# m13ammed/6D-Pose-Estimation-for-Unseen-Categories

Hardware: AMD Instinct MI355X
Metric: RGB-D crops/sec (fwd+bwd), 1024 pts, at 1/2/4/8 MI355X; pose err vs ref (higher is better)
Workload: dtype fp32; 1 GPU; configs[1] shape: B=32 synthetic 640x480 RGB-D crops, 1024 pts, training step fwd+bwd on 1 GPU (global batch 32); execution=hip-graph, crop formation overlapped, global_batch=32, points_per_crop=1024, cad_points=1024, precision=model fp32 (f32 MFMA); crop geometry / C_gt normal equations fp64, parallelism=dp1

## Files before the change

### 6d-pose-estimation-for-unseen-categories_amd/csrc/spectral.hip

```cpp
#include "common.hpp"
#include "mfma_tile.hpp"

namespace {

constexpr int kRows = 64;
constexpr int kKC = 64;

using pk::f32x4;

__device__ __forceinline__ f32x4 mfma4(float a, float b, f32x4 c) {
  return __builtin_amdgcn_mfma_f32_16x16x4f32(a, b, c, 0, 0, 0);
}

constexpr int kCPB = 4;
__global__ __launch_bounds__(256) void spec_reduce_mfma_kernel(const float* __restrict__ x, int ldx,
                                                               const float* __restrict__ mass,
                                                               const float* __restrict__ evecs, int N, int S,
                                                               float* __restrict__ part) {
  __shared__ float4 red[4][kKC * kKC / 4];
  const int s = blockIdx.x, b = blockIdx.y, tid = threadIdx.x;
  const int w = tid >> 6, l = tid & 63, u = l & 15, g = l >> 4;
  const float* __restrict__ phi = evecs + (int64_t)b * N * kKC;
  const float* __restrict__ xb = x + (int64_t)b * N * ldx;
  const float* __restrict__ mb = mass ? mass + (int64_t)b * N : nullptr;
  const int r0 = s * kCPB * kRows;
  const int nch = min(kCPB, (N - r0 + kRows - 1) / kRows);
  float4 pv[4], xv[4];
  float wv[4];
  auto load = [&](int ch) {
    const int rw = r0 + ch * kRows + 16 * w;
#pragma unroll
    for (int q = 0; q < 4; ++q) {
      const int r = rw + 4 * q + g;
      const int rc = r < N ? r : N - 1;
      pv[q] = reinterpret_cast<const float4*>(phi + (int64_t)rc * kKC)[u];
      xv[q] = reinterpret_cast<const float4*>(xb + (int64_t)rc * ldx)[u];
      wv[q] = mb ? mb[rc] : 1.f;
    }
  };
  f32x4 acc[4][4];
#pragma unroll
  for (int kt = 0; kt < 4; ++kt)
#pragma unroll
    for (int ct = 0; ct < 4; ++ct) acc[kt][ct] = f32x4{0.f, 0.f, 0.f, 0.f};
  load(0);
  for (int ch = 0; ch < nch; ++ch) {
    const int rw = r0 + ch * kRows + 16 * w;
    float a[4][4], xs[4][4];
#pragma unroll
    for (int q = 0; q < 4; ++q) {
      const bool ok = rw + 4 * q + g < N;
      const float wr = ok ? wv[q] : 0.f;
      a[q][0] = pv[q].x, a[q][1] = pv[q].y, a[q][2] = pv[q].z, a[q][3] = pv[q].w;
      xs[q][0] = mb ? xv[q].x * wr : (ok ? xv[q].x : 0.f);
      xs[q][1] = mb ? xv[q].y * wr : (ok ? xv[q].y : 0.f);
      xs[q][2] = mb ? xv[q].z * wr : (ok ? xv[q].z : 0.f);
      xs[q][3] = mb ? xv[q].w * wr : (ok ? xv[q].w : 0.f);
    }
    if (ch + 1 < nch) load(ch + 1);
#pragma unroll
    for (int q = 0; q < 4; ++q)
#pragma unroll
      for (int kt = 0; kt < 4; ++kt)
#pragma unroll
        for (int ct = 0; ct < 4; ++ct) acc[kt][ct] = mfma4(a[q][kt], xs[q][ct], acc[kt][ct]);
  }
#pragma unroll
  for (int kt = 0; kt < 4; ++kt)
#pragma unroll
    for (int rr = 0; rr < 4; ++rr)
      red[w][(4 * (4 * g + rr) + kt) * (kKC / 4) + u] =
          make_float4(acc[kt][0][rr], acc[kt][1][rr], acc[kt][2][rr], acc[kt][3][rr]);
  __syncthreads();
  float4* __restrict__ o = reinterpret_cast<float4*>(part + ((int64_t)b * S + s) * kKC * kKC);
#pragma unroll
  for (int j = 0; j < kKC * kKC / 4 / 256; ++j) {
    const int e = tid + 256 * j;
    const float4 v0 = red[0][e], v1 = red[1][e], v2 = red[2][e], v3 = red[3][e];
    o[e] = make_float4(((v0.x + v1.x) + v2.x) + v3.x, ((v0.y + v1.y) + v2.y) + v3.y, ((v0.z + v1.z) + v2.z) + v3.z,
                       ((v0.w + v1.w) + v2.w) + v3.w);
  }
}

__global__ __launch_bounds__(1024) void spec_combine4_kernel(float* __restrict__ part, int S,
                                                             const float* __restrict__ evals,
                                                             float* __restrict__ t, int clamp_t, int write_t,
                                                             float* __restrict__ raw, float* __restrict__ scaled,
                                                             const float* __restrict__ saved, int want_gt) {
  __shared__ double gsum[16][kKC];
  const int b = blockIdx.x, y = blockIdx.y, tid = threadIdx.x;
  const int c = tid & 63, k = 16 * y + (tid >> 6);
  const float* pb = part + (int64_t)b * S * kKC * kKC + k * kKC + c;
  const float tc = clamp_t ? fmaxf(t[c], 1e-8f) : t[c];
  double v = 0.0;
  int s = 0;
  for (; s + 8 <= S; s += 8) {
    float ld[8];
#pragma unroll
    for (int q = 0; q < 8; ++q) ld[q] = pb[(int64_t)(s + q) * kKC * kKC];
#pragma unroll
    for (int q = 0; q < 8; ++q) v += (double)ld[q];
  }
  for (; s < S; ++s) v += (double)pb[(int64_t)s * kKC * kKC];
  const float lam = evals[b * kKC + k];
  const float E = expf(-lam * tc);
  const int64_t o = (int64_t)b * kKC * kKC + k * kKC + c;
  const float vf = (float)v;
  if (raw) raw[o] = vf;
  scaled[o] = E * vf;
  if (write_t && b == 0 && y == 0 && tid < kKC) t[c] = tc;
  if (want_gt) {
    gsum[tid >> 6][c] = -(double)lam * (double)E * ((double)saved[o] * v);
    __syncthreads();
    if (tid < kKC) {
      double a = 0.0;
#pragma unroll
      for (int q = 0; q < 16; ++q) a += gsum[q][c];
      part[(int64_t)b * S * kKC * kKC + (16 * y) * kKC + c] = (float)a;
    }
  }
}

struct SpecFuse {
  const float* part;
  int S, clamp_t, write_t, pad;
  const float* evals;
  float* t;
  float* raw;
};

template <bool FUSED>
__global__ __launch_bounds__(256) void spec_expand_mfma_kernel(const float* __restrict__ evecs,
                                                               const float* __restrict__ coef,
                                                               const float* __restrict__ mass, int N,
                                                               float* __restrict__ y, int ldy, int accumulate,
                                                               const float* __restrict__ gtb, int64_t gt_stride,
                                                               float* __restrict__ gt, SpecFuse fz) {
  __shared__ float4 scoef[kKC * kKC / 4];
  const int3 lb = pk::xcd_block3();
  const int tile = lb.x, b = lb.y, tid = threadIdx.x;
  const int w = tid >> 6, l = tid & 63, u = l & 15, g = l >> 4;
  if constexpr (FUSED) {
    constexpr int PER = kKC * kKC / 4 / 256;
    const float* pb = fz.part + (int64_t)b * fz.S * kKC * kKC;
    double v[PER][4];
#pragma unroll
    for (int j = 0; j < PER; ++j)
#pragma unroll
      for (int q = 0; q < 4; ++q) v[j][q] = 0.0;
    for (int s0 = 0; s0 < fz.S; ++s0) {
      float4 ld[PER];
#pragma unroll
      for (int j = 0; j < PER; ++j) ld[j] = reinterpret_cast<const float4*>(pb + (int64_t)s0 * kKC * kKC)[tid + 256 * j];
#pragma unroll
      for (int j = 0; j < PER; ++j) {
        v[j][0] += (double)ld[j].x;
        v[j][1] += (double)ld[j].y;
        v[j][2] += (double)ld[j].z;
        v[j][3] += (double)ld[j].w;
      }
    }
#pragma unroll
    for (int j = 0; j < PER; ++j) {
      const int e = tid + 256 * j, k = e >> 4, c4 = e & 15;
      const float lam = fz.evals[b * kKC + k];
      float o[4], r[4];
#pragma unroll
      for (int q = 0; q < 4; ++q) {
        const int c = 4 * c4 + q;
        const float tc = fz.clamp_t ? fmaxf(fz.t[c], 1e-8f) : fz.t[c];
        const float E = expf(-lam * tc);
        r[q] = (float)v[j][q];
        o[q] = E * r[q];
      }
      scoef[e] = make_float4(o[0], o[1], o[2], o[3]);
      if (tile == 0 && fz.raw != nullptr)
        reinterpret_cast<float4*>(fz.raw + (int64_t)b * kKC * kKC)[e] = make_float4(r[0], r[1], r[2], r[3]);
    }
    if (fz.write_t && tile == 0 && b == 0 && tid < kKC) fz.t[tid] = fmaxf(fz.t[tid], 1e-8f);
  } else {
    const float* __restrict__ cb = coef + (int64_t)b * kKC * kKC;
    float4 cv[kKC * kKC / 4 / 256];
#pragma unroll
    for (int j = 0; j < kKC * kKC / 4 / 256; ++j) cv[j] = reinterpret_cast<const float4*>(cb)[tid + 256 * j];
#pragma unroll
    for (int j = 0; j < kKC * kKC / 4 / 256; ++j) scoef[tid + 256 * j] = cv[j];
  }
  const int rw = tile * 64 + 16 * w;
  const float* __restrict__ phi = evecs + (int64_t)b * N * kKC;
  float4 pv[4];
  {
    const int r = rw + u < N ? rw + u : N - 1;
#pragma unroll
    for (int t = 0; t < 4; ++t) pv[t] = reinterpret_cast<const float4*>(phi + (int64_t)r * kKC)[4 * t + g];
  }
  float wr[4];
  float4 old[4];
#pragma unroll
  for (int rr = 0; rr < 4; ++rr) {
    const int r = rw + 4 * g + rr < N ? rw + 4 * g + rr : N - 1;
    wr[rr] = mass ? mass[(int64_t)b * N + r] : 1.f;
    old[rr] = accumulate ? reinterpret_cast<const float4*>(y + ((int64_t)b * N + r) * ldy)[u]
                         : make_float4(0.f, 0.f, 0.f, 0.f);
  }
  __syncthreads();
  f32x4 acc[4];
#pragma unroll
  for (int ct = 0; ct < 4; ++ct) acc[ct] = f32x4{0.f, 0.f, 0.f, 0.f};
#pragma unroll
  for (int t = 0; t < 4; ++t) {
    const float pa[4] = {pv[t].x, pv[t].y, pv[t].z, pv[t].w};
#pragma unroll
    for (int e = 0; e < 4; ++e) {
      const float4 bv = scoef[(16 * t + 4 * g + e) * (kKC / 4) + u];
      acc[0] = mfma4(pa[e], bv.x, acc[0]);
      acc[1] = mfma4(pa[e], bv.y, acc[1]);
      acc[2] = mfma4(pa[e], bv.z, acc[2]);
      acc[3] = mfma4(pa[e], bv.w, acc[3]);
    }
  }
#pragma unroll
  for (int rr = 0; rr < 4; ++rr) {
    const int r = rw + 4 * g + rr;
    if (r >= N) continue;
    const float m = wr[rr];
    float4 v = make_float4(acc[0][rr] * m, acc[1][rr] * m, acc[2][rr] * m, acc[3][rr] * m);
    if (accumulate) {
      const float4 o = old[rr];
      v = make_float4(o.x + v.x, o.y + v.y, o.z + v.z, o.w + v.w);
    }
    reinterpret_cast<float4*>(y + ((int64_t)b * N + r) * ldy)[u] = v;
  }
  if (gt && tile == 0 && b == 0 && tid < kKC) {
    float a = 0.f;
    const int nq = (int)gridDim.y;
    for (int q0 = 0; q0 < nq; q0 += 8) {
      float v[8][4];
#pragma unroll
      for (int q = 0; q < 8; ++q) {
        const float* gq = gtb + (int64_t)(q0 + q < nq ? q0 + q : q0) * gt_stride + tid;
#pragma unroll
        for (int y = 0; y < 4; ++y) v[q][y] = gq[16 * kKC * y];
      }
#pragma unroll
      for (int q = 0; q < 8; ++q)
        if (q0 + q < nq) a += ((v[q][0] + v[q][1]) + v[q][2]) + v[q][3];
    }
    gt[tid] = a;
  }
}

}

extern "C" int pk_spectral_diffusion(const float* in, int ld_in, const float* mass, const float* evecs,
                                     const float* evals, float* t, int clamp_t, int B, int N, int K, int C,
                                     int mode, float* work, float* raw, float* scaled, const float* saved,
                                     float* gt, float* out, int ld_out, int accumulate, void* stream) {
  PK_REQUIRE(B >= 0 && N >= 0 && K == kKC && C == kKC && (mode == 0 || mode == 1));
  PK_REQUIRE(ld_in >= C && ld_out >= C && ld_in % 4 == 0 && ld_out % 4 == 0);
  if (B == 0 || N == 0) return PK_OK;
  PK_REQUIRE(in && evecs && evals && t && work && scaled && out);
  PK_REQUIRE(mode == 0 || (saved && gt));
  hipStream_t s = pk::as_stream(stream);
  const int S = (N + kCPB * kRows - 1) / (kCPB * kRows);
  hipLaunchKernelGGL(spec_reduce_mfma_kernel, dim3(S, B), dim3(256), 0, s, in, ld_in, mode == 0 ? mass : nullptr,
                     evecs, N, S, work);
  PK_CHECK_LAUNCH();
  if (mode == 0) {
    SpecFuse fz{work, S, clamp_t, (int)(clamp_t != 0), 0, evals, t, raw};
    hipLaunchKernelGGL(spec_expand_mfma_kernel<true>, dim3((N + 63) / 64, B), dim3(256), 0, s, evecs, scaled,
                       nullptr, N, out, ld_out, accumulate, work, (int64_t)S * kKC * kKC, nullptr, fz);
    PK_CHECK_LAUNCH();
    return PK_OK;
  }
  hipLaunchKernelGGL(spec_combine4_kernel, dim3(B, 4), dim3(1024), 0, s, work, S, evals, t, clamp_t, 0, raw, scaled,
                     saved, 1);
  PK_CHECK_LAUNCH();
  hipLaunchKernelGGL(spec_expand_mfma_kernel<false>, dim3((N + 63) / 64, B), dim3(256), 0, s, evecs, scaled, mass, N,
                     out, ld_out, accumulate, work, (int64_t)S * kKC * kKC, gt, SpecFuse{});
  PK_CHECK_LAUNCH();
  return PK_OK;
}
```

### 6d-pose-estimation-for-unseen-categories_amd/dpfm_amd/_lib.py

```python
from __future__ import annotations

import ctypes
import os
from typing import Optional

import torch

_HERE = os.path.dirname(os.path.abspath(__file__))
LIB_PATH = os.path.join(_HERE, "lib", "libposekern.so")
DEV_LIB_PATH = os.path.join(_HERE, "lib", "libposekern_dev.so")

_P = ctypes.c_void_p
_I = ctypes.c_int
_I64 = ctypes.c_int64
_U64 = ctypes.c_uint64
_D = ctypes.c_double
_F = ctypes.c_float



class LinearArgs(ctypes.Structure):
    _fields_ = [("x", _P), ("w", _P), ("bias", _P), ("layout", ctypes.c_int32), ("N", ctypes.c_int32),
                ("R", _I64), ("Cin", ctypes.c_int32), ("Cout", ctypes.c_int32), ("transw", ctypes.c_int32),
                ("act", ctypes.c_int32), ("mask", _P), ("ldx", _I64), ("y", _P), ("ldy", _I64), ("y2", _P),
                ("ldy2", _I64), ("split", ctypes.c_int32), ("store_cf", ctypes.c_int32), ("add", _P), ("lda", _I64),
                ("add_cols", ctypes.c_int32), ("pad", ctypes.c_int32), ("pre", _P), ("pre_out", _P),
                ("w2", _P), ("bias2", _P), ("wsplit", ctypes.c_int32), ("pad2", ctypes.c_int32), ("add2", _P),
                ("lda2", _I64)]


class OverlapHeadArgs(ctypes.Structure):
    _fields_ = [("x", _P * 2), ("strides", (_I64 * 3) * 2), ("N", ctypes.c_int32 * 2), ("B", ctypes.c_int32),
                ("pad", ctypes.c_int32), ("w0", _P), ("b0", _P), ("w1", _P), ("b1", _P), ("n", _P * 2),
                ("nrm", _P * 2), ("nrows", _P * 2), ("h", _P * 2), ("s", _P * 2), ("ds", _P * 2), ("dnr", _P * 2),
                ("g", _P * 2), ("dh", _P * 2), ("dx", _P * 2), ("dadd", _P * 2)]


SIGNATURES = {
    "pk_fps": [_P, _P, _I, _I, _P, _P, _P, _I, _P],
    "pk_ball_query_mask": [_P, _P, _P, _P, _P, _I, _I, _I, _P, _I, _P, _P],
    "pk_ball_query_pairs": [_P, _P, _P, _P, _P, _I, _I, _I, _P, _I, _P, _P, _P, _I64, _P, _P, _P, _P, _P, _P],
    "pk_backproject": [_P, _P, _I, _I, _I, _P, _P, _P, _P, _P, _P, _P, _I64, _P, _P, _P],
    "pk_sor": [_P, _P, _I, _I, _I, _D, _P, _P, _I, _I, _P, _P, _P, _P, _P, _P, _P, _P, _P, _P, _P],
    "pk_fps_npoint": [_P, _I, _I, _I, _U64, _I64, _P, _P, _P, _P],
    "pk_gather_transform": [_P, _P, _I, _P, _I, _P, _I, _P, _P, _P, _P, _P, _P, _P, _P],
    "pk_gather_transform_pad": [_P, _P, _I, _P, _I, _P, _I, _P, _P, _P, _P, _P, _P, _P, _I, _P, _P, _P, _P],
    "pk_collate_pad": [_P, _I, _I, _P, _I, _I, _P, _P, _P],
    "pk_segment_scan": [_P, _I, _I, _P, _P, _P],
    "pk_offsets_from_counts": [_P, _I, _P, _P],
    "pk_spectral_diffusion": [_P, _I, _P, _P, _P, _P, _I, _I, _I, _I, _I, _I, _P, _P, _P, _P, _P, _P, _I, _I, _P],
    "pk_linear_ex": [_P, _P],
    "pk_linear_ex2": [_P, _P, _P],
    "pk_fmap_head_work_len": [_I, _I, _I],
    "pk_fmap_head_fwd": [_P, _I, _P, _P, _P, _I, _P, _I, _P, _P, _P, _I, _P, _I, _P, _I, _I, _I, _I, _F, _P, _P, _P, _P,
                         _P, _P, _I64, _P],
    "pk_fmap_head_bwd": [_P, _P, _P, _P, _P, _I, _P, _I, _P, _I, _P, _I, _I, _I, _I, _P, _P, _P, _P, _P, _P, _P],
    "pk_fmap_solve": [_P, _P, _P, _F, _I, _I, _P, _P],
    "pk_fmap_solve_backward": [_P, _P, _P, _F, _I, _I, _P, _P, _P, _P],
    "pk_attention_fwd": [_P, _P, _P, _I, _I, _I, _I, _I, _I64, _I64, _P, _P, _P],
    "pk_attention_bwd": [_P, _P, _P, _P, _P, _P, _I, _I, _I, _I, _I, _I64, _I64, _P, _P, _P, _P, _I64, _I64, _P],
    "pk_attention_fwd_varlen": [_P, _P, _P, _I, _I, _I, _I, _I, _I64, _I64, _P, _P, _P, _P, _P],
    "pk_attention_bwd_varlen": [_P, _P, _P, _P, _P, _P, _I, _I, _I, _I, _I, _I64, _I64, _P, _P, _P, _P, _P, _P, _I64,
                                _I64, _P],
    "pk_linear_wgrad": [_P, _P, _I, _I64, _I, _I, _I, _P, _P, _P, _I, _P],
    "pk_linear_wgrad_grouped_work": [_P, _I],
    "pk_linear_wgrad_grouped": [_P, _I, _P, _I64, _P],
    "pk_nce_loss": [_P, _P, _P, _P, _I, _I64, _I64, _I, _P, _I, _P, _P, _I, _F, _I, _P, _P, _P, _P, _P, _P, _P],
    "pk_affine_cat": [_P, _I64, _P, _I64, _F, _F, _P, _P],
    "pk_loss_head": [_P, _P, _I, _I, _P, _P, _F, _F, _F, _P, _P, _P, _P],
    "pk_loss_scale": [_P, _P, _P, _P, _I, _P, _P],
    "pk_clip_rmsprop": [_P, _P, _P, _P, _P, _I, _F, _F, _F, _F, _F, _P, _P, _P],
    "pk_instnorm_relu_fwd": [_P, _I64, _I, _F, _P, _P, _P, _P],
    "pk_instnorm_relu_bwd": [_P, _P, _P, _P, _I64, _I, _P, _P],
    "pk_instnorm_relu_fwd_varlen": [_P, _I64, _I, _F, _P, _P, _P, _I, _P, _P],
    "pk_instnorm_relu_bwd_varlen": [_P, _P, _P, _P, _I64, _I, _P, _I, _P, _P],
    "pk_wbce": [_P, _P, _I, _P, _P, _I, _I, _P, _P, _P, _P],
    "pk_wbce_varlen": [_P, _P, _I, _P, _P, _I, _I, _P, _P, _P, _P, _P, _P],
    "pk_l2_normalize_fwd": [_P, _P, _I, _I, _I, _P, _P, _P, _P],
    "pk_l2_normalize_bwd": [_P, _P, _P, _P, _I, _I, _I, _P, _P, _P],
    "pk_overlap_head_fwd": [_P, _P],
    "pk_overlap_head_bwd": [_P, _P],
    "pk_mlp3_fwd": [_P, _I64, _P, _I64, _P, _P, _P, _P, _P, _P, _I64, _I, _P, _P, _P, _I64, _I, _P],
    "pk_mlp3_bwd": [_P, _P, _P, _P, _P, _P, _I64, _I, _P, _P, _P, _P, _I, _P],
    "pk_attn_mlp_fwd": [_P, _P, _P, _P, _P, _P, _I, _I, _I, _F, _P, _P, _P, _P, _P, _P],
    "pk_attn_mlp_bwd_norm": [_P, _P, _P, _P, _P, _I, _I, _I, _P, _P],
    "pk_attn_mlp_bwd_in": [_P, _P, _P, _I, _I, _I, _P, _P, _P],
    "pk_resolvent_mask": [_P, _I, _P, _I, _I, _I, _F, _P, _P],
    "pk_linear_fwd": [_P, _P, _P, _I, _I64, _I, _I, _I, _I, _I, _P, _P, _P],
    "pk_feat_dist_work_size": [_I, _I, _I, _I, _I],
    "pk_attention_bwd_work_size": [_I, _I, _I, _I, _I],
    "pk_feat_dist_topk": [_P, _I, _P, _P, _I, _P, _P, _I, _I, _I, _I, _I, _P, _I64, _P, _P, _P],
    "pk_rigidity_filter_work_size": [_I, _I, _I],
    "pk_rigidity_filter": [_P, _I, _P, _P, _I, _P, _I, _P, _I, _I, _P, _P, _P, _P, _P, _P, _P],
    "pk_inlier_ratio": [_P, _I, _I, _P, _P, _I, _P, _I, _P, _I, _P, _P, _P],
    "pk_cgt_lstsq_work_size": [_I, _I, _I],
    "pk_nce_select": [_P, _I, _I64, _I, ctypes.c_uint64, _P, _P, _P, _P],
    "pk_cgt_lstsq": [_P, _I, _P, _P, _I, _I, _P, _I, _I, _I, _I, _P, _I, _P, _P, _P],
    "pk_ransac_work_size": [_I, _I64, _I],
    "pk_ransac": [_P, _P, _P, _P, _P, _P, _P, _P, _U64, _I64, _D, _I, _I, _P, _I64, _P, _P, _P, _P],
    "pk_pose_metrics": [_P, _P, _I, _I, _P, _P, _P, _P, _P],
    "pk_bop_errors": [_P, _P, _I, _I, _P, _P, _P, _P, _P, _I, _P, _P, _P, _P],
    "pk_erode_mask": [_P, _I, _I, _I, _P, _P],
    "pk_sample_rgb": [_P, _I, _I, _I, _I, _P, _P, _P, _I, _P, _P],
    "pk_sample_features": [_P, _I, _I, _I, _I, _P, _P, _P, _I, _P, _P],
    "pk_icp_work_size": [_I, _I, _I],
    "pk_icp_init": [_P, _P, _P, _P, _P, _I, _I, _I, _P, _I64, _P],
    "pk_icp_iterate": [_P, _P, _P, _P, _D, _I, _D, _D, _I, _I, _I, _I, _P, _I64, _P, _P],
    "pk_icp_result": [_P, _I, _P, _P, _P],
    "pk_icp": [_P, _P, _P, _P, _P, _D, _I, _D, _D, _I, _I, _I, _I, _P, _I64, _P, _P, _P, _P],
    "pk_normals_work_size": [_I, _I],
    "pk_estimate_normals": [_P, _P, _I, _I, _I, _D, _D, _D, _P, _P, _P, _I64, _P],
    "pk_icp_plane_work_size": [_I, _I, _I],
    "pk_icp_plane_init": [_P, _P, _P, _P, _P, _P, _I, _I, _I, _P, _I64, _P],
    "pk_icp_plane_iterate": [_P, _P, _P, _P, _D, _I, _D, _D, _I, _I, _I, _I, _P, _I64, _P, _P],
    "pk_teaser_graph": [_P, _P, _P, _I, _I, _D, _P, _P, _P],
    "pk_knn": [_P, _P, _I, _I, _I, _I, _P, _P, _P],
    "pk_pc_local_tri": [_P, _P, _I, _I, _P, _I, _P, _P, _P, _P],
    "pk_cotan_dense": [_P, _P, _I, _I, _P, _P, _I, _P, _P, _I, _D, _D, _P, _P, _P],
    "pk_sym_scale": [_P, _I, _I, _D, _P, _D, _P, _P],
    "pk_dgemm_cheb": [_P, _P, _P, _I, _I, _I, _D, _D, _D, _P, _P],
    "pk_dgemm_tn": [_P, _P, _I, _I, _I, _P, _P],
    "pk_dpotrf": [_P, _I, _I, _D, _P, _P],
    "pk_dpotrs": [_P, _P, _I, _I, _I, _P],
    "pk_tufted_laplacian": [_P, _I64, _P, _I64, _D, _I64, _P, _P, _P, _P, _P, _P],
    "pk_grad_build": [_P, _P, _I, _I, _P, _P, _I, _P, _P, _P],
    "pk_grad_apply": [_P, _I64, _P, _P, _I, _I, _I, _I, _P, _P],
    "pk_grad_apply_t": [_P, _P, _P, _P, _I, _I, _I, _I, _P, _I64, _I, _P],
    "pk_gradfeat_fwd": [_P, _P, _P, _I64, _I, _P, _I64, _P],
    "pk_gradfeat_bwd": [_P, _I64, _P, _I64, _P, _P, _P, _I64, _I, _P, _P, _P],
    "pk_linear192_fwd": [_P, _I64, _P, _P, _I64, _I, _P, _P],
    "pk_teaser_solve": [_P, _P, _P, _I, _I, _P, _P, _P, _I, _P, _P, _P, _P],
    "pk_teaser_scale_work_size": [_I, _I],
    "pk_teaser_scale": [_P, _P, _P, _I, _I, _D, _P, _I64, _P, _P, _P],
    "pk_teaser_graph_scaled": [_P, _P, _P, _I, _I, _D, _P, _P, _P, _P],
    "pk_teaser_solve_scaled": [_P, _P, _P, _I, _I, _P, _P, _P, _I, _P, _P, _P, _P, _P],
    "pk_transpose_cf_rows": [_P, _P, _I, _I, _I, _I, _I64, _P, _P],
    "pk_mean_f32": [_P, _I64, _P, _P],
    "pk_copy_rows": [_P, _I64, _P, _I64, _I64, _I64, _P],
    "pk_device_cu_count": [_P],
    "pk_stream_create_cu_mask": [_P, _I, _P],
    "pk_stream_get_cu_mask": [_P, _I, _P],
    "pk_stream_destroy": [_P],
    "pk_build_id": [_P, _I],
}

RESTYPES = {"pk_cgt_lstsq_work_size": _I64, "pk_linear_wgrad_grouped_work": _I64, "pk_ransac_work_size": _I64,
            "pk_feat_dist_work_size": _I64, "pk_fmap_head_work_len": _I64, "pk_icp_work_size": _I64,
            "pk_rigidity_filter_work_size": _I64, "pk_attention_bwd_work_size": _I64,
            "pk_normals_work_size": _I64, "pk_icp_plane_work_size": _I64,
            "pk_teaser_scale_work_size": _I64}

_lib: Optional[ctypes.CDLL] = None
_dev_lib: Optional[ctypes.CDLL] = None


class WgradCall(ctypes.Structure):
    _fields_ = [("x", _P), ("dy", _P), ("dw", _P), ("db", _P), ("R", _I64), ("I", ctypes.c_int32),
                ("O", ctypes.c_int32), ("N", ctypes.c_int32), ("layout", ctypes.c_int32),
                ("accumulate", ctypes.c_int32), ("pad", ctypes.c_int32), ("sx", _I64), ("sdy", _I64)]


class TeaserParams(ctypes.Structure):
    _fields_ = [("noise_bound", _D), ("cbar2", _D), ("rotation_gnc_factor", _D), ("rotation_cost_threshold", _D),
                ("kcore_heuristic_threshold", _D), ("rotation_max_iterations", ctypes.c_int32),
                ("pad", ctypes.c_int32), ("max_clique_nodes", _I64)]


class PoseKernError(RuntimeError):
    pass


def lib() -> ctypes.CDLL:
    global _lib
    if _lib is None:
        if not os.path.exists(LIB_PATH):
            raise PoseKernError(
                f"libposekern.so not found at {LIB_PATH}: build it with "
                "`make -C 6d-pose-estimation-for-unseen-categories_amd` (no CPU fallback exists)")
        l = ctypes.CDLL(LIB_PATH, mode=ctypes.RTLD_GLOBAL)
        for name, argtypes in SIGNATURES.items():
            fn = getattr(l, name)
            fn.argtypes = argtypes
            fn.restype = RESTYPES.get(name, ctypes.c_int)
        _lib = l
    return _lib


def dev_lib() -> ctypes.CDLL:
    global _dev_lib
    if _dev_lib is None:
        if not os.path.exists(DEV_LIB_PATH):
            raise PoseKernError(f"libposekern_dev.so not found at {DEV_LIB_PATH}: `make -C "
                                "6d-pose-estimation-for-unseen-categories_amd`")
        l = ctypes.CDLL(DEV_LIB_PATH, mode=ctypes.RTLD_LOCAL)
        for name, argtypes in SIGNATURES.items():
            fn = getattr(l, name)
            fn.argtypes = argtypes
            fn.restype = RESTYPES.get(name, ctypes.c_int)
        _dev_lib = l
    return _dev_lib


def use_dev_lib() -> None:
    global _lib
    if _lib is not None and _lib is not dev_lib():
        raise PoseKernError("use_dev_lib() must run before the first library call")
    _lib = dev_lib()


_ERRORS = {1000: "invalid argument", 1001: "output capacity exceeded"}
_probe = None


def build_id(l: Optional[ctypes.CDLL] = None) -> str:
    buf = ctypes.create_string_buffer(65)
    st = (l or lib()).pk_build_id(buf, 65)
    if st != 0:
        raise PoseKernError(f"pk_build_id failed: {st}")
    return buf.value.decode()


def tree_build_id() -> str:
    import glob
    import hashlib
    pkg = os.path.dirname(_HERE)
    names = sorted([os.path.relpath(f, pkg) for pat in ("*.hip", "*.hpp", "*.cpp")
                    for f in glob.glob(os.path.join(pkg, "csrc", pat))] + ["../include/posekern.h", "Makefile"])
    h = hashlib.sha256()
    for n in names:
        with open(os.path.join(pkg, n), "rb") as f:
            h.update(f.read())
    return h.hexdigest()


def set_probe(hook) -> None:
    global _probe
    _probe = hook


def call(name: str, *args, work=None) -> None:
    fn = getattr(lib(), name)
    status = _probe(name, lambda: fn(*args), work) if _probe is not None else fn(*args)
    if status != 0:
        msg = _ERRORS.get(status, f"hipError_t {status}")
        raise PoseKernError(f"{name} failed: {msg}")


def ptr(t: Optional[torch.Tensor]):
    if t is None:
        return None
    if not t.is_cuda:
        raise PoseKernError("posekern ops take HIP device tensors only (no CPU fallback)")
    if not t.is_contiguous():
        raise PoseKernError("posekern ops need contiguous tensors")
    return ctypes.c_void_p(t.data_ptr())


def stream(device: torch.device):
    return ctypes.c_void_p(torch.cuda.current_stream(device).cuda_stream)
```

### include/posekern.h

```cpp
#ifndef POSEKERN_H
#define POSEKERN_H
#include <stdint.h>

#ifdef __cplusplus
extern "C" {
#endif

int pk_fps(const float* xyz, const int64_t* off, int B, int nmax, const int32_t* start,
           const int32_t* npoint, int64_t* out, int out_stride, void* stream);

int pk_ball_query_mask(const double* cad, const int64_t* cad_off, const double* pc,
                       const int64_t* pc_off, const double* thr2, int B, int n1max, int n2max,
                       uint8_t* mask, int ld, int32_t* rowcount, void* stream);

int pk_ball_query_pairs(const double* cad, const int64_t* cad_off, const double* pc,
                        const int64_t* pc_off, const double* thr2, int B, int n1max, int n2max,
                        const uint8_t* mask, int ld, const int32_t* rowcount, int64_t* rowoff,
                        int64_t* pairs, int64_t cap, int64_t* count, int8_t* ov12, int8_t* ov21,
                        int32_t* over, int32_t* colcount, void* stream);

int pk_backproject(const uint16_t* depth, const uint8_t* mask, int F, int H, int W,
                   const double* K, const float* cam_scale, int32_t* rowcnt, int64_t* rowoff,
                   int64_t* count, int64_t* off, double* xyz, int64_t cap, int32_t* pix,
                   int32_t* idxmap, void* stream);

int pk_sor(const double* xyz, const int64_t* off, int B, int nmax, int knn, double std_ratio,
           const int32_t* pix, const int32_t* idxmap, int H, int W, const double* K, double* avg,
           double* thr,
           int32_t* ccount, int64_t* coff, int64_t* kept, int64_t* out_off, double* out64,
           float* out32, int64_t* kept_idx, void* stream);

int pk_fps_npoint(const int64_t* off, int B, int fixed, int limit, uint64_t seed, int64_t base,
                  int32_t* npoint, int32_t* start, int64_t* out_off, void* stream);

int pk_gather_transform(const double* pcd, const int64_t* off, int B, const int64_t* idx,
                        int idx_stride, const int32_t* npoint, int npmax, const int64_t* out_off,
                        const double* R, const double* t, double* sel64, double* align64,
                        float* sel32, int32_t* status, void* stream);

int pk_gather_transform_pad(const double* pcd, const int64_t* off, int B, const int64_t* idx,
                            int idx_stride, const int32_t* npoint, int npmax, const int64_t* out_off,
                            const double* R, const double* t, double* sel64, double* align64,
                            float* sel32, int32_t* status, int ld, float* pad_sel32, float* pad_align32,
                            int32_t* counts, void* stream);

int pk_collate_pad(const void* src, int src_f64, int C, const int64_t* off, int B, int ld, float* dst,
                   int32_t* counts, void* stream);

int pk_segment_scan(const int32_t* cnt, int S, int n, int64_t* off, int64_t* total, void* stream);
int pk_offsets_from_counts(const int64_t* counts, int B, int64_t* off, void* stream);

int pk_spectral_diffusion(const float* in, int ld_in, const float* mass, const float* evecs, const float* evals,
                          float* t, int clamp_t, int B, int N, int K, int C, int mode, float* work, float* raw,
                          float* scaled, const float* saved, float* gt, float* out, int ld_out, int accumulate,
                          void* stream);

int pk_fmap_solve(const float* AAt, const float* BAt, const float* D, float lambda, int B, int K,
                  float* C, void* stream);
int pk_fmap_solve_backward(const float* AAt, const float* BAt, const float* D, float lambda, int B,
                           int K, const float* G, float* dBAt, float* dAAt_part, void* stream);

int pk_attention_fwd(const float* q, const float* k, const float* v, int B, int D, int H, int N,
                     int M, int64_t sbk, int64_t sbv, float* out, float* lse, void* stream);
int64_t pk_attention_bwd_work_size(int B, int D, int H, int N, int M);
int pk_attention_bwd(const float* q, const float* k, const float* v, const float* out,
                     const float* dout, const float* lse, int B, int D, int H, int N, int M,
                     int64_t sbk, int64_t sbv, float* work, float* dq, float* dk, float* dv, int64_t sbdk,
                     int64_t sbdv, void* stream);
int pk_attention_fwd_varlen(const float* q, const float* k, const float* v, int B, int D, int H, int N,
                            int M, int64_t sbk, int64_t sbv, const int* qlen, const int* klen, float* out,
                            float* lse, void* stream);
int pk_attention_bwd_varlen(const float* q, const float* k, const float* v, const float* out,
                            const float* dout, const float* lse, int B, int D, int H, int N, int M,
                            int64_t sbk, int64_t sbv, const int* qlen, const int* klen, float* work, float* dq,
                            float* dk, float* dv, int64_t sbdk, int64_t sbdv, void* stream);

int pk_linear_wgrad(const float* x, const float* dy, int layout, int64_t R, int I, int O, int N,
                    float* work, float* dw, float* db, int accumulate, void* stream);

typedef struct pk_wgrad_call {
  const float* x;
  const float* dy;
  float* dw;
  float* db;
  int64_t R;
  int32_t I, O, N, layout, accumulate, pad;
  int64_t sx, sdy;
} pk_wgrad_call;
int64_t pk_linear_wgrad_grouped_work(const pk_wgrad_call* calls, int n);
int pk_linear_wgrad_grouped(const pk_wgrad_call* calls, int n, float* work, int64_t work_elems, void* stream);

int pk_clip_rmsprop(float* const* params, float* const* grads, float* const* square_avg, float* const* steps,
                    const int64_t* numel, int n, float max_norm, float lr, float alpha, float one_minus_alpha,
                    float eps, float* work, float* norm_out, void* stream);

int pk_instnorm_relu_fwd(const float* x, int64_t rows, int N, float eps, float* y, float* mean, float* invstd,
                         void* stream);
int pk_instnorm_relu_bwd(const float* x, const float* dy, const float* mean, const float* invstd, int64_t rows,
                         int N, float* dx, void* stream);
int pk_instnorm_relu_fwd_varlen(const float* x, int64_t rows, int N, float eps, float* y, float* mean,
                                float* invstd, int C, const int* lens, void* stream);
int pk_instnorm_relu_bwd_varlen(const float* x, const float* dy, const float* mean, const float* invstd,
                                int64_t rows, int N, float* dx, int C, const int* lens, void* stream);

int pk_wbce(const float* p12, const int8_t* t12, int N1, const float* p21, const int8_t* t21, int N2, int B,
            float* loss, float* g12, float* g21, void* stream);
int pk_wbce_varlen(const float* p12, const int8_t* t12, int N1, const float* p21, const int8_t* t21, int N2,
                   int B, const int* n1, const int* n2, float* loss, float* g12, float* g21, void* stream);

int pk_affine_cat(const float* a, int64_t na, const float* b, int64_t nb, float sub, float mul, float* out,
                  void* stream);

int pk_l2_normalize_fwd(const float* x, const int64_t* strides, int B, int N, int C, float* y, float* nrm,
                        float* y_rows, void* stream);
int pk_l2_normalize_bwd(const float* y, const float* dy, const float* nrm, const int64_t* strides, int B, int N,
                        int C, float* dx, const float* dy_rows, void* stream);

typedef struct pk_overlap_head_args {
  const float* x[2];
  int64_t strides[2][3];
  int32_t N[2];
  int32_t B, pad;
  const float* w0;
  const float* b0;
  const float* w1;
  const float* b1;
  float* n[2];
  float* nrm[2];
  float* nrows[2];
  float* h[2];
  float* s[2];
  const float* ds[2];
  const float* dnr[2];
  float* g[2];
  float* dh[2];
  float* dx[2];
  const float* dadd[2];
} pk_overlap_head_args;
int pk_overlap_head_fwd(const pk_overlap_head_args* a, void* stream);
int pk_overlap_head_bwd(const pk_overlap_head_args* a, void* stream);

int pk_mlp3_fwd(const float* x_in, int64_t ld_in, const float* x_diff, int64_t ld_diff, const float* w1,
                const float* b1, const float* w2, const float* b2, const float* w3, const float* b3, int64_t R, int C,
                float* h1, float* h2, float* y, int64_t ldy, int max_blocks, void* stream);
int pk_mlp3_bwd(const float* dy, const float* h2, const float* h1, const float* w3, const float* w2, const float* w1,
                int64_t R, int C, float* d2, float* d1, float* dx, float* dd, int max_blocks, void* stream);

int pk_attn_mlp_fwd(const float* x, const float* a, const float* wm, const float* bm, const float* w0,
                    const float* b0, int B, int C, int N, float eps, float* hc, float* h1, float* h1n, float* mean,
                    float* invstd, void* stream);
int pk_attn_mlp_bwd_norm(const float* dout, const float* w3, const float* h1, const float* mean, const float* invstd,
                         int B, int C, int N, float* dh1, void* stream);
int pk_attn_mlp_bwd_in(const float* dh1, const float* w0, const float* wm, int B, int C, int N, float* dhc, float* da,
                       void* stream);

int64_t pk_fmap_head_work_len(int B, int N1, int N2);
int pk_fmap_head_fwd(const float* evecs_x, int ldex, const float* mass_x, const float* fx, const int64_t* fx_strides,
                     int N1, const float* evecs_y, int ldey, const float* mass_y, const float* fy,
                     const int64_t* fy_strides, int N2, const float* evals_x, int ldvx, const float* evals_y, int ldvy,
                     int B, int K, int C, float gamma, float* A, float* Bm, float* AAt, float* BAt, float* D,
                     float* work, int64_t work_len, void* stream);
int pk_fmap_head_bwd(const float* part, const float* dBAt, const float* A, const float* Bm, const float* evecs_x,
                     int ldex, const float* mass_x, int N1, const float* evecs_y, int ldey, const float* mass_y, int N2,
                     int B, int K, int C, float* dA, float* dBm, float* dfx, const int64_t* dfx_strides, float* dfy,
                     const int64_t* dfy_strides, void* stream);

int pk_resolvent_mask(const float* evals1, int ld1, const float* evals2, int ld2, int B, int K, float gamma, float* D,
                      void* stream);

int pk_linear_fwd(const float* x, const float* w, const float* bias, int layout, int64_t R, int N, int Cin,
                  int Cout, int transw, int relu, const float* mask, float* y, void* stream);

typedef struct pk_linear_args {
  const float* x;
  const float* w;
  const float* bias;
  int32_t layout;
  int32_t N;
  int64_t R;
  int32_t Cin, Cout, transw, act;
  const float* mask;
  int64_t ldx;
  float* y;
  int64_t ldy;
  float* y2;
  int64_t ldy2;
  int32_t split, store_cf;
  const float* add;
  int64_t lda;
  int32_t add_cols, pad;
  const float* pre;
  float* pre_out;
  const float* w2;
  const float* bias2;
  int32_t wsplit, pad2;
  const float* add2;
  int64_t lda2;
} pk_linear_args;
int pk_linear_ex(const pk_linear_args* a, void* stream);
int pk_linear_ex2(const pk_linear_args* a0, const pk_linear_args* a1, void* stream);

int64_t pk_feat_dist_work_size(int B, int V1max, int V2max, int topk, int mode);
int pk_feat_dist_topk(const float* evecs_x, int ldx, const float* C, const float* evecs_y, int ldy,
                      const int32_t* n1, const int32_t* n2, int B, int V1max, int V2max, int topk, int mode,
                      void* work, int64_t work_bytes, int64_t* out_idx, float* out_dist, void* stream);

int64_t pk_rigidity_filter_work_size(int B, int nmax, int ldc);
int pk_rigidity_filter(const int64_t* cand, int ldc, const int32_t* ncand, const float* cad, int ldcad,
                       const float* pc, int ldpc, const float* thr4, int B, int nmax, int64_t* list_a,
                       int64_t* list_b, int32_t* n_a, int32_t* n_b, float* score, float* partial, void* stream);

int pk_inlier_ratio(const int64_t* pairs, int ldp, int layout, const int32_t* npairs, const float* cad,
                    int ldcad, const float* pc_aligned, int ldpc, const float* thr, int B, float* ir,
                    int32_t* status, void* stream);
int pk_mean_f32(const float* x, int64_t n, float* out, void* stream);

int64_t pk_cgt_lstsq_work_size(int ldp, int V2max, int B);

int pk_nce_select(const int64_t* count, int B, int64_t cap, int num, uint64_t seed, int64_t* ctr,
                  int64_t* rows, uint8_t* valid, void* stream);
int pk_nce_loss(const float* f1, const int64_t* st1, const float* f2, const int64_t* st2, int B, int64_t N1,
                int64_t N2, int C, const int64_t* pairs,
                int cap, const int64_t* rows, const uint8_t* valid, int S, float nce_t, int prenorm, float* lse,
                float* term, float* loss, float* g1, float* g2, float* dx_rows, void* stream);

int pk_loss_head(const float* C12, const float* Cgt, int B, int K, const float* nce, const float* wb,
                 float w_fmap, float w_acc, float w_nce, float* loss, float* logs, float* dC, void* stream);
int pk_loss_scale(const float* const* src, float* const* dst, const int64_t* numel, const float* scale, int n,
                  const float* g, void* stream);
int pk_cgt_lstsq(const int64_t* pairs, int ldp, const int64_t* npairs, const float* evecs1, int ld1,
                 int V1max, const float* evecs2, int ld2, int V2max, int B, int K, const int32_t* cnt,
                 int ldc, double* work, float* Cgt, void* stream);

int64_t pk_ransac_work_size(int B, int64_t H, int nmax);
int pk_ransac(const double* src, const int64_t* src_off, const double* dst, const int64_t* dst_off,
              const int32_t* corres, const int64_t* cor_off, const int32_t* hyps, const int64_t* hyp_off,
              uint64_t seed, int64_t H, double max_dist, int B, int nmax, void* work, int64_t work_bytes,
              double* T, double* stats, int32_t* status, void* stream);

int pk_pose_metrics(const double* cad, const int64_t* off, int B, int nmax, const double* T_est,
                    const double* T_gt, double* work, double* out, void* stream);

#define PK_BOP_QUERY_BLOCK 512
#define PK_BOP_TARGET_TILE 1024
#define PK_BOP_SYM_CHUNK 8
int pk_bop_errors(const double* cad, const int64_t* off, int B, int nmax, const double* T_est,
                  const double* T_gt, const double* K, const double* sym, const int64_t* sym_off, int smax,
                  double* work, double* out, int32_t* best, void* stream);

int pk_erode_mask(const uint8_t* mask, int F, int H, int W, uint8_t* out, void* stream);

int pk_sample_rgb(const uint8_t* img, int F, int H, int W, int C, const double* K, const double* pts,
                  const int64_t* off, int nmax, float* out, void* stream);

int pk_sample_features(const float* fmap, int F, int C, int H, int W, const double* K, const double* pts,
                       const int64_t* off, int nmax, float* out, void* stream);

int64_t pk_icp_work_size(int B, int nsrc_max, int ntgt_max);
int pk_icp_init(const double* src, const int64_t* src_off, const double* tgt, const int64_t* tgt_off,
                const double* T_init, int B, int nsrc_max, int ntgt_max, void* work, int64_t work_bytes, void* stream);
int pk_icp_iterate(const double* src, const int64_t* src_off, const double* tgt, const int64_t* tgt_off,
                   double max_dist, int max_iter, double rel_fitness, double rel_rmse, int B, int nsrc_max,
                   int ntgt_max, int steps, void* work, int64_t work_bytes, int32_t* active_count, void* stream);
int pk_icp_result(const void* work, int B, double* T, double* stats, void* stream);
int pk_icp(const double* src, const int64_t* src_off, const double* tgt, const int64_t* tgt_off, const double* T_init,
           double max_dist, int max_iter, double rel_fitness, double rel_rmse, int B, int nsrc_max, int ntgt_max,
           int poll, void* work, int64_t work_bytes, int32_t* dev_count, double* T, double* stats, void* stream);

int64_t pk_normals_work_size(int B, int nmax);
int pk_estimate_normals(const double* pts, const int64_t* off, int B, int nmax, int k, double vx, double vy, double vz,
                        double* normals, int32_t* knn, void* work, int64_t work_bytes, void* stream);

int64_t pk_icp_plane_work_size(int B, int nsrc_max, int ntgt_max);
int pk_icp_plane_init(const double* src, const int64_t* src_off, const double* tgt, const int64_t* tgt_off,
                      const double* tgt_normals, const double* T_init, int B, int nsrc_max, int ntgt_max, void* work,
                      int64_t work_bytes, void* stream);
int pk_icp_plane_iterate(const double* src, const int64_t* src_off, const double* tgt, const int64_t* tgt_off,
                         double max_dist, int max_iter, double rel_fitness, double rel_rmse, int B, int nsrc_max,
                         int ntgt_max, int steps, void* work, int64_t work_bytes, int32_t* active_count, void* stream);

typedef struct pk_teaser_params {
  double noise_bound;
  double cbar2;
  double rotation_gnc_factor;
  double rotation_cost_threshold;
  double kcore_heuristic_threshold;
  int32_t rotation_max_iterations;
  int32_t pad;
  int64_t max_clique_nodes;
} pk_teaser_params;
int pk_teaser_graph(const double* src, const double* dst, const int64_t* off, int B, int nmax, double beta,
                    uint64_t* adj, int32_t* deg, void* stream);
int pk_teaser_solve(const double* src, const double* dst, const int64_t* off, int B, int nmax, const uint64_t* adj,
                    const int32_t* deg, const pk_teaser_params* params, int threads, double* T, int32_t* clique,
                    int32_t* clique_size, int32_t* info);

int64_t pk_teaser_scale_work_size(int B, int nmax);
int pk_teaser_scale(const double* src, const double* dst, const int64_t* off, int B, int nmax, double beta,
                    void* work, int64_t work_bytes, double* scale, int32_t* scale_info, void* stream);
int pk_teaser_graph_scaled(const double* src, const double* dst, const int64_t* off, int B, int nmax, double beta,
                           const double* scale, uint64_t* adj, int32_t* deg, void* stream);
int pk_teaser_solve_scaled(const double* src, const double* dst, const int64_t* off, int B, int nmax,
                           const uint64_t* adj, const int32_t* deg, const pk_teaser_params* params, int threads,
                           const double* scale, double* T, int32_t* clique, int32_t* clique_size, int32_t* info);

int pk_knn(const double* pts, const int64_t* off, int B, int nmax, int k, int omit_self, int32_t* idx, double* d2,
           void* stream);
int pk_pc_local_tri(const double* pts, const int64_t* off, int B, int nmax, const int32_t* knn, int k, int32_t* tri,
                    int32_t* ntri, double* normals, void* stream);
int pk_cotan_dense(const double* pts, const int64_t* off, int B, int nmax, const int32_t* tri, const int32_t* ntri,
                   int k, const int32_t* faces, const int64_t* foff, int fmax, double scale, double denom_eps,
                   double* L, double* mass, void* stream);
int pk_sym_scale(const int64_t* off, int B, int nmax, double eps, const double* mass, double pad_diag, double* A,
                 void* stream);
int pk_dgemm_cheb(const double* A, const double* Y, const double* X, int B, int n, int m, double alpha, double beta,
                  double gamma, double* out, void* stream);
int pk_dgemm_tn(const double* X, const double* Y, int B, int n, int m, double* G, void* stream);
int pk_dpotrf(double* A, int B, int n, double tau, int32_t* fail, void* stream);
int pk_dpotrs(const double* L, double* X, int B, int n, int m, void* stream);
int pk_tufted_laplacian(const double* pts, int64_t n, const int32_t* tri, int64_t ntri, double mollify_factor,
                        int64_t cap, int32_t* ii, int32_t* jj, double* ww, int64_t* nnz, double* mass,
                        int64_t* nflips);

int pk_grad_build(const double* pts, const int64_t* off, int B, int nmax, const double* frames, const int32_t* nbr,
                  int W, int32_t* idx, double* val, void* stream);

int pk_grad_apply(const float* x, int64_t ldx, const int32_t* idx, const float* val, int B, int N, int W, int C,
                  float* v, void* stream);
int pk_grad_apply_t(const float* dv, const int32_t* tptr, const int32_t* tsrc, const float* val, int B, int N, int W,
                    int C, float* dx, int64_t lddx, int accumulate, void* stream);
int pk_gradfeat_fwd(const float* v, const float* A_re, const float* A_im, int64_t R, int C, float* g, int64_t ldg,
                    void* stream);
int pk_gradfeat_bwd(const float* dg, int64_t lddg, const float* g, int64_t ldg, const float* v, const float* A_re,
                    const float* A_im, int64_t R, int C, float* dv, float* pq, void* stream);
int pk_linear192_fwd(const float* x, int64_t ldx, const float* w, const float* bias, int64_t R, int relu, float* y,
                     void* stream);

int pk_copy_rows(float* dst, int64_t ld_dst, const float* src, int64_t ld_src, int64_t rows, int64_t n,
                 void* stream);

int pk_transpose_cf_rows(const float* src0, const float* src1, int B0, int B, int C, int N, int64_t sb,
                         float* dst, void* stream);

int pk_device_cu_count(int* out);
int pk_stream_create_cu_mask(const uint32_t* mask, int words, void** stream);
int pk_stream_get_cu_mask(void* stream, int words, uint32_t* mask);
int pk_stream_destroy(void* stream);

int pk_build_id(char* out, int cap);

#ifdef __cplusplus
}
#endif
#endif
```

Measured before the change: 19760 crops/s.

## Fuse spectral reduce and coefficient combine into one channel-split kernel for backward

Adds a fused spectral diffusion kernel. Each block owns 16 channels of one batch item and walks all rows with software-pipelined loads and MFMA. Partial sums are reduced in shared memory with fp64 accumulation, and the exp(-lambda t) scaling and t-gradient terms are computed in the same kernel. A planner picks this path by CU count and N; on the default path the backward pass uses the fused reduce plus the existing expand kernel, replacing the separate reduce and combine launches. The gain is one fewer launch and no global partial buffer, but each block now reads the eigenvectors per channel group, and the forward pass keeps the old three-pass code.

Result: no change. 19830 crops/s, median of 6 (+0.3%).

```diff
diff --git a/6d-pose-estimation-for-unseen-categories_amd/csrc/spectral.hip b/6d-pose-estimation-for-unseen-categories_amd/csrc/spectral.hip
--- a/6d-pose-estimation-for-unseen-categories_amd/csrc/spectral.hip
+++ b/6d-pose-estimation-for-unseen-categories_amd/csrc/spectral.hip
@@ -1,3 +1,5 @@
+#include <atomic>
+
 #include "common.hpp"
 #include "mfma_tile.hpp"
 
@@ -250,19 +252,289 @@
   }
 }
 
-}
-
-extern "C" int pk_spectral_diffusion(const float* in, int ld_in, const float* mass, const float* evecs,
-                                     const float* evals, float* t, int clamp_t, int B, int N, int K, int C,
-                                     int mode, float* work, float* raw, float* scaled, const float* saved,
-                                     float* gt, float* out, int ld_out, int accumulate, void* stream) {
+constexpr int kCG = 16;
+constexpr int kFW = 8;
+template <int MODE, bool EXPAND>
+__global__ __launch_bounds__(64 * kFW, 4) void spec_fused_kernel(
+    const float* __restrict__ in, int ldx, const float* __restrict__ mass, const float* __restrict__ evecs,
+    const float* __restrict__ evals, float* t, int clamp_t, int N, int S, float* __restrict__ raw,
+    const float* __restrict__ saved, float* __restrict__ gtb, float* __restrict__ y, int ldy, int accumulate,
+    float* __restrict__ scaled, int64_t gt_stride) {
+  constexpr int NT = 64 * kFW, SPR = kFW / 4, PER = kKC * kCG / NT, TR = 3;
+  constexpr int kSlab = kCPB * kRows, kPart = kKC * kCG;
+  __shared__ __attribute__((aligned(16))) float red[kFW * kPart];
+  __shared__ float scoef[kPart];
+  __shared__ float pre[(1 + 2 * PER) * NT];
+  const int3 lb = pk::xcd_block3();
+  const int c0 = lb.x * kCG, b = lb.y, tid = threadIdx.x;
+  const int wv = __builtin_amdgcn_readfirstlane(tid >> 6), l = tid & 63, u = l & 15, g = l >> 4;
+  const int w = wv & 3, sl = wv >> 2;
+  const float* __restrict__ phi = evecs + (int64_t)b * N * kKC;
+  const float* __restrict__ xb = in + (int64_t)b * N * ldx + c0 + u;
+  const float* __restrict__ mb = (MODE == 0 && mass) ? mass + (int64_t)b * N : nullptr;
+
+  struct Chunk {
+    float4 pv[4];
+    float xv[4];
+  };
+  auto load = [&](Chunk& c, int s, int ch) {
+    const int rw = s * kSlab + ch * kRows + 16 * w;
+#pragma unroll
+    for (int q = 0; q < 4; ++q) {
+      const int r = rw + 4 * q + g;
+      const int rc = r < N ? r : N - 1;
+      c.pv[q] = reinterpret_cast<const float4*>(phi + (int64_t)rc * kKC)[u];
+      c.xv[q] = xb[(int64_t)rc * ldx];
+    }
+  };
+  auto load_mass = [&](int s) {
+    const int r = s * kSlab + (l >> 4) * kRows + 16 * w + (l & 15);
+    return mb[r < N ? r : N - 1];
+  };
+  f32x4 acc[4];
+  auto compute = [&](const Chunk& c, int s, int ch, float mreg) {
+    const int rw = s * kSlab + ch * kRows + 16 * w;
+#pragma unroll
+    for (int q = 0; q < 4; ++q) {
+      const bool ok = rw + 4 * q + g < N;
+      float xs;
+      if (mb) {
+        const float m = __shfl(mreg, 16 * ch + 4 * q + g);
+        const float wr = ok ? m : 0.f;
+        xs = c.xv[q] * wr;
+      } else {
+        xs = ok ? c.xv[q] : 0.f;
+      }
+      const float a[4] = {c.pv[q].x, c.pv[q].y, c.pv[q].z, c.pv[q].w};
+#pragma unroll
+      for (int kt = 0; kt < 4; ++kt) acc[kt] = mfma4(a[kt], xs, acc[kt]);
+    }
+  };
+  auto chunks_of = [&](int s) { return s < S ? min(kCPB, (N - s * kSlab + kRows - 1) / kRows) : 0; };
+
+  double v[PER];
+#pragma unroll
+  for (int j = 0; j < PER; ++j) v[j] = 0.0;
+  Chunk cb[kCPB];
+  int s = sl, nch = chunks_of(s);
+  float mcur = 0.f, mnext = 0.f;
+#pragma unroll
+  for (int ch = 0; ch < kCPB; ++ch)
+    if (ch < nch) load(cb[ch], s, ch);
+  if (mb && nch > 0) mcur = load_mass(s);
+  static_assert(NT % kCG == 0, "a thread's coefficients share their channel");
+  pre[tid] = t[c0 + tid % kCG];
+#pragma unroll
+  for (int j = 0; j < PER; ++j) {
+    const int e = tid + NT * j, k = e / kCG, c = c0 + e % kCG;
+    pre[NT * (1 + j) + tid] = evals[b * kKC + k];
+    if constexpr (MODE == 1) pre[NT * (1 + PER + j) + tid] = saved[(int64_t)b * kKC * kKC + k * kKC + c];
+  }
+  const int rounds = (S + SPR - 1) / SPR;
+  for (int rd = 0; rd < rounds; ++rd) {
+    const int s_next = s + SPR, nch_next = chunks_of(s_next);
+    if (mb && nch_next > 0) mnext = load_mass(s_next);
+#pragma unroll
+    for (int kt = 0; kt < 4; ++kt) acc[kt] = f32x4{0.f, 0.f, 0.f, 0.f};
+#pragma unroll
+    for (int ch = 0; ch < kCPB; ++ch) {
+      if (ch < nch) compute(cb[ch], s, ch, mcur);
+      if (ch < nch_next) load(cb[ch], s_next, ch);
+    }
+    if (nch > 0) {
+      float* rw = red + wv * kPart + u;
+#pragma unroll
+      for (int kt = 0; kt < 4; ++kt)
+#pragma unroll
+        for (int rr = 0; rr < 4; ++rr) rw[(4 * (4 * g + rr) + kt) * kCG] = acc[kt][rr];
+    }
+    s = s_next, nch = nch_next, mcur = mnext;
+    __syncthreads();
+#pragma unroll
+    for (int q = 0; q < SPR; ++q) {
+      if (rd * SPR + q >= S) break;
+      const float* rq = red + 4 * q * kPart;
+#pragma unroll
+      for (int j = 0; j < PER; ++j) {
+        const int e = tid + NT * j;
+        const float p = ((rq[e] + rq[kPart + e]) + rq[2 * kPart + e]) + rq[3 * kPart + e];
+        v[j] += (double)p;
+      }
+    }
+    __syncthreads();
+  }
+
+  int tq = tid;
+  asm volatile("" : "+v"(tq));
+  const int u2 = tq & 15, g2 = (tq >> 4) & 3;
+
+  const float* __restrict__ mrow = (MODE == 1 && mass) ? mass + (int64_t)b * N : nullptr;
+  float* __restrict__ yb = y + (int64_t)b * N * ldy + c0 + u2;
+  struct Tile {
+    float4 pv[4];
+    float wr[4];
+    float old[4];
+  };
+  auto load_tile = [&](Tile& tl, int rw) {
+    const int r = rw + u2 < N ? rw + u2 : N - 1;
+#pragma unroll
+    for (int t4 = 0; t4 < 4; ++t4) tl.pv[t4] = reinterpret_cast<const float4*>(phi + (int64_t)r * kKC)[4 * t4 + g2];
+#pragma unroll
+    for (int rr = 0; rr < 4; ++rr) {
+      const int r2 = rw + 4 * g2 + rr < N ? rw + 4 * g2 + rr : N - 1;
+      tl.wr[rr] = mrow ? mrow[r2] : 1.f;
+      tl.old[rr] = accumulate ? yb[(int64_t)r2 * ldy] : 0.f;
+    }
+  };
+  Tile tb[TR];
+  if constexpr (EXPAND) {
+#pragma unroll
+    for (int i = 0; i < TR; ++i)
+      if (16 * (wv + kFW * i) < N) load_tile(tb[i], 16 * (wv + kFW * i));
+  }
+
+  double* gs = reinterpret_cast<double*>(red);
+#pragma unroll
+  for (int j = 0; j < PER; ++j) {
+    const int e = tq + NT * j, k = e / kCG, c = c0 + e % kCG;
+    const float tt = pre[tq], lam = pre[NT * (1 + j) + tq];
+    const float tc = clamp_t ? fmaxf(tt, 1e-8f) : tt;
+    const float E = expf(-lam * tc);
+    const int64_t o = (int64_t)b * kKC * kKC + k * kKC + c;
+    const float vf = (float)v[j];
+    if (raw) raw[o] = vf;
+    if constexpr (EXPAND) scoef[e] = E * vf;
+    else scaled[o] = E * vf;
+    if constexpr (MODE == 1) gs[e] = -(double)lam * (double)E * ((double)pre[NT * (1 + PER + j) + tq] * v[j]);
+  }
+  if (MODE == 0 && clamp_t && b == 0 && tq < kCG) t[c0 + tq] = fmaxf(pre[tq], 1e-8f);
+  __syncthreads();
+  if constexpr (MODE == 1) {
+    if (tq < kCG) {
+      float f[4];
+#pragma unroll
+      for (int yy = 0; yy < 4; ++yy) {
+        double a = 0.0;
+#pragma unroll
+        for (int q = 0; q < 16; ++q) a += gs[(16 * yy + q) * kCG + tq];
+        f[yy] = (float)a;
+      }
+      const float gv = ((f[0] + f[1]) + f[2]) + f[3];
+      if constexpr (EXPAND) {
+        gtb[b * kKC + c0 + tq] = gv;
+      } else {
+#pragma unroll
+        for (int yy = 0; yy < 4; ++yy) gtb[b * gt_stride + 16 * kKC * yy + c0 + tq] = yy == 0 ? gv : 0.f;
+      }
+    }
+  }
+  if constexpr (!EXPAND) return;
+
+  float bc[16];
+#pragma unroll
+  for (int i = 0; i < 16; ++i) bc[i] = scoef[(16 * (i >> 2) + 4 * g2 + (i & 3)) * kCG + u2];
+  for (int rw0 = 16 * wv; rw0 < N; rw0 += 16 * kFW * TR) {
+#pragma unroll
+    for (int i = 0; i < TR; ++i) {
+      const int rw = rw0 + 16 * kFW * i;
+      if (rw >= N) break;
+      const Tile& cur = tb[i];
+      f32x4 o = f32x4{0.f, 0.f, 0.f, 0.f};
+#pragma unroll
+      for (int t4 = 0; t4 < 4; ++t4) {
+        const float pa[4] = {cur.pv[t4].x, cur.pv[t4].y, cur.pv[t4].z, cur.pv[t4].w};
+#pragma unroll
+        for (int e = 0; e < 4; ++e) o = mfma4(pa[e], bc[4 * t4 + e], o);
+      }
+#pragma unroll
+      for (int rr = 0; rr < 4; ++rr) {
+        const int r = rw + 4 * g2 + rr;
+        if (r >= N) continue;
+        float res = o[rr] * cur.wr[rr];
+        if (accumulate) res = cur.old[rr] + res;
+        yb[(int64_t)r * ldy] = res;
+      }
+      if (rw + 16 * kFW * TR < N) load_tile(tb[i], rw + 16 * kFW * TR);
+    }
+  }
+}
+
+__global__ __launch_bounds__(64) void spec_gt_sum_kernel(const float* __restrict__ gtb, int B,
+                                                         float* __restrict__ gt) {
+  const int tid = threadIdx.x;
+  float a = 0.f;
+  for (int q0 = 0; q0 < B; q0 += 8) {
+    float v[8];
+#pragma unroll
+    for (int q = 0; q < 8; ++q) v[q] = gtb[(int64_t)(q0 + q < B ? q0 + q : q0) * kKC + tid];
+#pragma unroll
+    for (int q = 0; q < 8; ++q)
+      if (q0 + q < B) a += v[q];
+  }
+  gt[tid] = a;
+}
+
+constexpr int kPathThreePass = 1, kPathFused = 2, kPathFusedReduce = 3;
+
+int spec_plan(int B, int N, int cus) {
+  if (cus <= 0) cus = 256;
+  return ((int64_t)B * (kKC / kCG) * 4 >= cus && N <= 1024) ? kPathFusedReduce : kPathThreePass;
+}
+
+int device_cus() {
+  static std::atomic<int> known[16];
+  int dev = 0, cus = 0;
+  if (hipGetDevice(&dev) != hipSuccess) return 0;
+  const bool slot = dev >= 0 && dev < 16;
+  if (slot && (cus = known[dev].load(std::memory_order_relaxed)) > 0) return cus;
+  if (hipDeviceGetAttribute(&cus, hipDeviceAttributeMultiprocessorCount, dev) != hipSuccess) return 0;
+  if (slot) known[dev].store(cus, std::memory_order_relaxed);
+  return cus;
+}
+
+}
+
+extern "C" int pk_spectral_plan(int B, int N, int cus) { return spec_plan(B, N, cus); }
+
+extern "C" int pk_spectral_diffusion_ex(const float* in, int ld_in, const float* mass, const float* evecs,
+                                        const float* evals, float* t, int clamp_t, int B, int N, int K, int C,
+                                        int mode, float* work, float* raw, float* scaled, const float* saved,
+                                        float* gt, float* out, int ld_out, int accumulate, void* stream,
+                                        int path) {
   PK_REQUIRE(B >= 0 && N >= 0 && K == kKC && C == kKC && (mode == 0 || mode == 1));
   PK_REQUIRE(ld_in >= C && ld_out >= C && ld_in % 4 == 0 && ld_out % 4 == 0);
+  PK_REQUIRE(path >= 0 && path <= 3);
   if (B == 0 || N == 0) return PK_OK;
   PK_REQUIRE(in && evecs && evals && t && work && scaled && out);
   PK_REQUIRE(mode == 0 || (saved && gt));
   hipStream_t s = pk::as_stream(stream);
   const int S = (N + kCPB * kRows - 1) / (kCPB * kRows);
+  if (path == 0) path = spec_plan(B, N, device_cus());
+  if (path == kPathFused) {
+    const dim3 grid(kKC / kCG, B), block(64 * kFW);
+    if (mode == 0)
+      hipLaunchKernelGGL((spec_fused_kernel<0, true>), grid, block, 0, s, in, ld_in, mass, evecs, evals, t, clamp_t, N,
+                         S, raw, saved, work, out, ld_out, accumulate, nullptr, 0);
+    else
+      hipLaunchKernelGGL((spec_fused_kernel<1, true>), grid, block, 0, s, in, ld_in, mass, evecs, evals, t, clamp_t, N,
+                         S, raw, saved, work, out, ld_out, accumulate, nullptr, 0);
+    PK_CHECK_LAUNCH();
+    if (mode == 1) {
+      hipLaunchKernelGGL(spec_gt_sum_kernel, dim3(1), dim3(64), 0, s, work, B, gt);
+      PK_CHECK_LAUNCH();
+    }
+    return PK_OK;
+  }
+  if (path == kPathFusedReduce && mode == 1) {
+    hipLaunchKernelGGL((spec_fused_kernel<1, false>), dim3(kKC / kCG, B), dim3(64 * kFW), 0, s, in, ld_in, mass,
+                       evecs, evals, t, clamp_t, N, S, raw, saved, work, out, ld_out, accumulate, scaled,
+                       (int64_t)S * kKC * kKC);
+    PK_CHECK_LAUNCH();
+    hipLaunchKernelGGL(spec_expand_mfma_kernel<false>, dim3((N + 63) / 64, B), dim3(256), 0, s, evecs, scaled, mass,
+                       N, out, ld_out, accumulate, work, (int64_t)S * kKC * kKC, gt, SpecFuse{});
+    PK_CHECK_LAUNCH();
+    return PK_OK;
+  }
   hipLaunchKernelGGL(spec_reduce_mfma_kernel, dim3(S, B), dim3(256), 0, s, in, ld_in, mode == 0 ? mass : nullptr,
                      evecs, N, S, work);
   PK_CHECK_LAUNCH();
@@ -281,3 +553,11 @@
   PK_CHECK_LAUNCH();
   return PK_OK;
 }
+
+extern "C" int pk_spectral_diffusion(const float* in, int ld_in, const float* mass, const float* evecs,
+                                     const float* evals, float* t, int clamp_t, int B, int N, int K, int C,
+                                     int mode, float* work, float* raw, float* scaled, const float* saved,
+                                     float* gt, float* out, int ld_out, int accumulate, void* stream) {
+  return pk_spectral_diffusion_ex(in, ld_in, mass, evecs, evals, t, clamp_t, B, N, K, C, mode, work, raw, scaled,
+                                  saved, gt, out, ld_out, accumulate, stream, 0);
+}
diff --git a/6d-pose-estimation-for-unseen-categories_amd/dpfm_amd/_lib.py b/6d-pose-estimation-for-unseen-categories_amd/dpfm_amd/_lib.py
--- a/6d-pose-estimation-for-unseen-categories_amd/dpfm_amd/_lib.py
+++ b/6d-pose-estimation-for-unseen-categories_amd/dpfm_amd/_lib.py
@@ -49,6 +49,9 @@
     "pk_segment_scan": [_P, _I, _I, _P, _P, _P],
     "pk_offsets_from_counts": [_P, _I, _P, _P],
     "pk_spectral_diffusion": [_P, _I, _P, _P, _P, _P, _I, _I, _I, _I, _I, _I, _P, _P, _P, _P, _P, _P, _I, _I, _P],
+    "pk_spectral_diffusion_ex": [_P, _I, _P, _P, _P, _P, _I, _I, _I, _I, _I, _I, _P, _P, _P, _P, _P, _P, _I, _I, _P,
+                                 _I],
+    "pk_spectral_plan": [_I, _I, _I],
     "pk_linear_ex": [_P, _P],
     "pk_linear_ex2": [_P, _P, _P],
     "pk_fmap_head_work_len": [_I, _I, _I],
diff --git a/include/posekern.h b/include/posekern.h
--- a/include/posekern.h
+++ b/include/posekern.h
@@ -54,6 +54,11 @@
                           float* t, int clamp_t, int B, int N, int K, int C, int mode, float* work, float* raw,
                           float* scaled, const float* saved, float* gt, float* out, int ld_out, int accumulate,
                           void* stream);
+int pk_spectral_diffusion_ex(const float* in, int ld_in, const float* mass, const float* evecs, const float* evals,
+                             float* t, int clamp_t, int B, int N, int K, int C, int mode, float* work, float* raw,
+                             float* scaled, const float* saved, float* gt, float* out, int ld_out, int accumulate,
+                             void* stream, int path);
+int pk_spectral_plan(int B, int N, int cus);
 
 int pk_fmap_solve(const float* AAt, const float* BAt, const float* D, float lambda, int B, int K,
                   float* C, void* stream);
```
